# Lymphatus/caesium-clt

Hardware: NVIDIA H100
Metric: megapixels/sec JPEG q=80 4K re-encode (higher is better)
Workload: dtype i32

## Files before the change

### caesium-clt_b200/csrc/jpeg_device.cu

```cuda
#include <cuda_runtime.h>
#include <malloc.h>
#include <chrono>
#include <cstdio>
#include <cstdlib>
#include <algorithm>
#include <condition_variable>
#include <cstring>
#include <mutex>
#include <vector>
#include <atomic>
#include "jpeg_device.h"
#include "resize_kernels.h"
#include "jpeg_gpuenc.h"
#include "jpeg_gpudec.h"
#include "png_device.h"
#include "webp_device.h"
#include "vp8l_device.h"
#include "gif_device.h"
#include "stream_wait.h"
#include "launch_timer.h"

namespace b200 {

thread_local LaunchTimer *tl_launch_timer = nullptr;

static constexpr size_t align_up(size_t v, size_t a) { return (v + a - 1) / a * a; }

bool plan_image(const JpegGeom &gin, const JpegGeom &gout, ImagePlan &p, std::string &err)
{
    p = ImagePlan();
    if (gin.ncomp != gout.ncomp || gin.width != gout.width || gin.height != gout.height) { err = "geometry mismatch between decode and encode side"; return false; }
    p.in_bytes = (size_t)gin.total_coefs * 2; p.out_bytes = (size_t)gout.total_coefs * 2;
    size_t off_plane = 0, off_full = 0, off_d = 0;
    for (int c = 0; c < gin.ncomp; c++) {
        if (gin.hmax % gin.hs[c] || gin.vmax % gin.vs[c] || gout.hmax % gout.hs[c] || gout.vmax % gout.vs[c]) { err = "fractional sampling ratio unsupported"; return false; }
        int uhx = gin.hmax / gin.hs[c], uvx = gin.vmax / gin.vs[c], dhx = gout.hmax / gout.hs[c], dvx = gout.vmax / gout.vs[c];
        if (uhx == 1 && uvx == 1 && dhx == 1 && dvx == 1) p.path[c] = PATH_FUSED;
        else if (uhx == 2 && uvx == 2 && dhx == 2 && dvx == 2) p.path[c] = PATH_C420;
        else p.path[c] = PATH_GENERIC;
        if (p.path[c] != PATH_FUSED) { p.plane_off[c] = off_plane; off_plane += align_up((size_t)gin.bw[c] * 8 * gin.bh[c] * 8, 256); }
        if (p.path[c] == PATH_GENERIC) {
            p.full_off[c] = off_full; off_full += align_up((size_t)gin.width * gin.height, 256);
            p.dplane_off[c] = off_d; off_d += align_up((size_t)gout.rbw[c] * 8 * gout.rbh[c] * 8, 256);
        }
    }
    p.plane_bytes = off_plane; p.full_bytes = off_full; p.dplane_bytes = off_d;
    return true;
}

void append_image_work(const JpegGeom &gin, const JpegGeom &gout, const ImagePlan &plan,
                       const int16_t *d_in, int16_t *d_out, uint8_t *d_scratch,
                       const uint16_t *d_dq, const QuantDev *d_q, WorkLists &wl)
{
    for (int c = 0; c < gin.ncomp; c++) {
        CompWork w; memset(&w, 0, sizeof(w));
        w.cin = d_in + gin.comp_offset[c]; w.cout = d_out + gout.comp_offset[c];
        w.dq = d_dq + 64 * c; w.q = d_q + gout.tq[c];
        w.bw_in = gin.bw[c]; w.bh_in = gin.bh[c]; w.rbw_in = gin.rbw[c]; w.rbh_in = gin.rbh[c]; w.cw = gin.cw[c]; w.ch = gin.ch[c];
        w.bw_out = gout.bw[c]; w.bh_out = gout.bh[c]; w.rbw_out = gout.rbw[c]; w.rbh_out = gout.rbh[c];
        w.W = gin.width; w.H = gin.height;
        w.pstride = gin.bw[c] * 8; w.fstride = gin.width;
        w.up_hx = gin.hmax / gin.hs[c]; w.up_vx = gin.vmax / gin.vs[c];
        w.dn_hx = gout.hmax / gout.hs[c]; w.dn_vx = gout.vmax / gout.vs[c];
        if (plan.path[c] != PATH_FUSED) w.plane = d_scratch + plan.plane_off[c];
        if (plan.path[c] == PATH_GENERIC) {
            w.full = d_scratch + plan.plane_bytes + plan.full_off[c];
            w.dplane = d_scratch + plan.plane_bytes + plan.full_bytes + plan.dplane_off[c];
        }
        const int t_in = work_tiles(w.rbw_in, w.rbh_in), t_out = work_tiles(w.rbw_out, w.rbh_out);
        switch (plan.path[c]) {
            case PATH_FUSED: wl.fused.push_back(w); wl.max_fused = std::max(wl.max_fused, t_out); break;
            case PATH_C420:
                wl.idct.push_back(w); wl.max_idct = std::max(wl.max_idct, t_in);
                wl.c420.push_back(w); wl.max_c420 = std::max(wl.max_c420, t_out);
                break;
            default:
                wl.idct.push_back(w); wl.max_idct = std::max(wl.max_idct, t_in);
                wl.up.push_back(w); wl.max_up_w = std::max(wl.max_up_w, w.W); wl.max_up_h = std::max(wl.max_up_h, w.H);
                wl.down.push_back(w); wl.max_dn_w = std::max(wl.max_dn_w, w.rbw_out * 8); wl.max_dn_h = std::max(wl.max_dn_h, w.rbh_out * 8);
                wl.fdct.push_back(w); wl.max_fdct = std::max(wl.max_fdct, t_out);
        }
    }
}

size_t flatten_work(const WorkLists &wl, CompWork *h)
{
    size_t n = 0;
    for (const auto *v : {&wl.fused, &wl.idct, &wl.c420, &wl.up, &wl.down, &wl.fdct, &wl.trel}) { if (!v->empty()) memcpy(h + n, v->data(), v->size() * sizeof(CompWork)); n += v->size(); }
    return n;
}
// ... 147 lines not shown
bool Slot::ensure(size_t in_bytes, size_t out_bytes, size_t scratch_bytes, size_t par_bytes, std::string &err)
{
    return h_in.reserve(in_bytes, Grow::Slot, err) && h_out.reserve(out_bytes, Grow::Slot, err) &&
           ensure_device(in_bytes, out_bytes, scratch_bytes, par_bytes, err);
}

static constexpr size_t par_dq_off = align_up(sizeof(QuantDev) * 4, 256);
static size_t par_work_off(int K) { return par_dq_off + align_up(sizeof(uint16_t) * 256 * K, 256); }
static constexpr size_t par_trellis_bytes = 256 + sizeof(JtTable) * 4;
static size_t put_trellis(Slot *s, const JpegGeom &gout, size_t end, WorkLists &wl)
{
    const size_t off = align_up(end, 256);
    JtTable *t = reinterpret_cast<JtTable *>(s->h_par + off);
    for (int i = 0; i < 4; i++) if (gout.qt_present[i]) jt_make_table(gout.qt[i], i != 0, &t[i]);
    add_trellis_work(wl);
    wl.trel_q = reinterpret_cast<const QuantDev *>(s->d_par.get());
    wl.trel_t = reinterpret_cast<const JtTable *>(s->d_par + off);
    return off + sizeof(JtTable) * 4;
}

static void put_quant(Slot *s, const JpegGeom &gout)
{
    QuantDev *q = reinterpret_cast<QuantDev *>(s->h_par.get());
    for (int t = 0; t < 4; t++) if (gout.qt_present[t]) make_quant_dev(gout.qt[t], &q[t]);
}
static const QuantDev *dev_quant(const Slot *s) { return reinterpret_cast<const QuantDev *>(s->d_par.get()); }
static const uint16_t *put_dequant(Slot *s, int k, const JpegGeom &gin)
{
    uint16_t *dq = reinterpret_cast<uint16_t *>(s->h_par + par_dq_off) + 256 * k;
    for (int c = 0; c < gin.ncomp; c++) memcpy(dq + 64 * c, gin.qt[gin.tq[c]], 128);
    return reinterpret_cast<const uint16_t *>(s->d_par + par_dq_off) + 256 * k;
}

static bool fill_transform_params(Slot *s, const JpegGeom *const *gins, const JpegGeom &gout, const GroupLayout &L, bool trellis, WorkLists &wl,
                                  size_t &par_bytes, size_t &work_off, std::string &err)
{
    put_quant(s, gout);
    wl.clear();
    for (int k = 0; k < L.K; k++) {
        const JpegGeom &gin = *gins[k];
        ImagePlan plan;
        if (!plan_image(gin, gout, plan, err)) return false;
        append_image_work(gin, gout, plan, L.coefs(*s, k, true), L.coefs(*s, k, false), s->d_scratch + L.scratch_stride * k,
                          put_dequant(s, k, gin), dev_quant(s), wl);
    }
    work_off = par_work_off(L.K);
    if (!trellis) { par_bytes = work_off + flatten_work(wl, reinterpret_cast<CompWork *>(s->h_par + work_off)) * sizeof(CompWork); return true; }
    const size_t end = work_off + (wl.total() + wl.fused.size() + wl.c420.size() + wl.fdct.size()) * sizeof(CompWork);
    par_bytes = put_trellis(s, gout, end, wl);
    flatten_work(wl, reinterpret_cast<CompWork *>(s->h_par + work_off));
    return true;
}

bool slot_transform(Slot *s, const JpegGeom &gin, const JpegGeom &gout, std::string &err, bool download, bool upload)
{
    ImagePlan plan;
    if (!plan_image(gin, gout, plan, err)) return false;
    cudaStream_t st = (cudaStream_t)s->stream;
    if (!s->ensure(plan.in_bytes, plan.out_bytes, plan.scratch_bytes(), par_work_off(1) + sizeof(CompWork) * 4 * 7 + par_trellis_bytes, err)) return false;
    GroupLayout L; L.K = 1;
    const JpegGeom *gins = &gin;
    WorkLists wl; size_t pbytes = 0, work_off = 0;
    if (!fill_transform_params(s, &gins, gout, L, jpeg_trellis(), wl, pbytes, work_off, err)) return false;
    CU(cudaMemcpyAsync(s->d_par, s->h_par, pbytes, cudaMemcpyHostToDevice, st));
    if (upload) CU(cudaMemcpyAsync(s->d_in, s->h_in, plan.in_bytes, cudaMemcpyHostToDevice, st));
    const int rc = launch_work(wl, reinterpret_cast<const CompWork *>(s->d_par + work_off), st);
    if (!launch_ok(rc, "kernel launch", err)) return false;
    if (!download) return true;
    CU(cudaMemcpyAsync(s->h_out, s->d_out, plan.out_bytes, cudaMemcpyDeviceToHost, st));
    CU(stream_wait(st));
    return true;
}

bool slot_group_layout(Slot *s, const JpegGeom &gin, const JpegGeom &gout, int K, GroupLayout &L, std::string &err)
{
    ImagePlan plan;
    if (!plan_image(gin, gout, plan, err)) return false;
    L.K = K;
    L.in_stride = align_up(plan.in_bytes, 256); L.out_stride = align_up(plan.out_bytes, 256); L.scratch_stride = align_up(std::max<size_t>(plan.scratch_bytes(), 256), 256);
    const size_t par = par_work_off(K) + sizeof(CompWork) * (size_t)K * 4 * 7 + 256 + par_trellis_bytes;
    return s->ensure_device(L.in_stride * K, L.out_stride * K, L.scratch_stride * K, par, err);
}

bool slot_transform_group_prepare(Slot *s, const JpegGeom *const *gins, const JpegGeom &gout, const GroupLayout &L, bool trellis, std::string &err)
{
    return fill_transform_params(s, gins, gout, L, trellis, s->group_wl, s->group_par_bytes, s->group_work_off, err);
}
bool slot_transform_group_enqueue(Slot *s, std::string &err)
{
    cudaStream_t st = (cudaStream_t)s->stream;
    CU(cudaMemcpyAsync(s->d_par, s->h_par, s->group_par_bytes, cudaMemcpyHostToDevice, st));
    const int rc = launch_work(s->group_wl, reinterpret_cast<const CompWork *>(s->d_par + s->group_work_off), st);
    if (!launch_ok(rc, "kernel launch", err)) return false;
    return true;
}
bool slot_transform_group(Slot *s, const JpegGeom *const *gins, const JpegGeom &gout, const GroupLayout &L, bool trellis, std::string &err)
{
    return slot_transform_group_prepare(s, gins, gout, L, trellis, err) && slot_transform_group_enqueue(s, err);
}

static std::atomic<long long> g_grp_ns[5];
static std::atomic<long long> g_grp_n{0};
static const bool g_grp_trace = getenv("B200_TRACE") != nullptr;
static void print_group_trace()
{
    const long long n = g_grp_n.load();
    if (!g_grp_trace || !n) return;
    static const char *names[] = {"stage inputs (memcpy to pinned, tables, H2D enqueue)", "enqueue decode + transform + encode (launch overhead)", "wait: sizes (GPU still busy)", "wait: final (after D2H enqueue)", "whole megabatch on the host"};
    fprintf(stderr, "[b200 trace] %lld megabatches; mean host ms per megabatch:\n", n);
    for (int i = 0; i < 5; i++) fprintf(stderr, "[b200 trace]   %-58s %8.3f\n", names[i], g_grp_ns[i].load() / 1e6 / (double)n);
}

static bool graphs_enabled() { static const bool on = [] { const char *e = getenv("B200_GRAPHS"); return !(e && !strcmp(e, "0")); }(); return on; }
static void drop_graphs(Slot *s)
{
    if (s->graph_front) { cudaGraphExecDestroy((cudaGraphExec_t)s->graph_front); s->graph_front = nullptr; }
    if (s->graph_back) { cudaGraphExecDestroy((cudaGraphExec_t)s->graph_back); s->graph_back = nullptr; }
    s->graph_sig = 0;
}
template <class Fn> static bool capture_graph(cudaStream_t st, void *&exec_out, Fn fn, std::string &err)
{
    if (cudaStreamBeginCapture(st, cudaStreamCaptureModeThreadLocal) != cudaSuccess) { cudaGetLastError(); return false; }
    const bool ok = fn();
    cudaGraph_t g = nullptr;
    const cudaError_t e = cudaStreamEndCapture(st, &g);
    if (!ok || e != cudaSuccess || !g) { if (g) cudaGraphDestroy(g); cudaGetLastError(); if (err.empty()) err = "graph capture failed"; return false; }
    cudaGraphExec_t ex = nullptr;
    const cudaError_t ei = cudaGraphInstantiate(&ex, g, 0);
    cudaGraphDestroy(g);
    if (ei != cudaSuccess) { cudaGetLastError(); err = std::string("cudaGraphInstantiate: ") + cudaGetErrorString(ei); return false; }
    exec_out = ex;
    return true;
}

bool slot_run_group(Slot *s, std::vector<GpuDecoder::Item> &items, const JpegGeom *const *gins, const JpegGeom &gout, const GroupLayout &L, bool progressive,
                    bool lossless, std::string &err)
{
    cudaStream_t st = (cudaStream_t)s->stream;
    const auto t0 = std::chrono::steady_clock::now();
    if (!s->decoder()->prepare(items, st, err)) return false;
    if (!lossless && !slot_transform_group_prepare(s, gins, gout, L, jpeg_trellis(), err)) return false;
    std::vector<int16_t *> bases((size_t)L.K);
    for (int k = 0; k < L.K; k++) bases[k] = L.coefs(*s, k, lossless);
    if (!s->encoder()->prepare(gout, progressive, bases.data(), L.K, st, s->dec->raw_bytes(), err)) return false;
    const auto t1 = std::chrono::steady_clock::now();
    auto front = [&]() { return s->dec->upload(st, err) && s->dec->enqueue(st, err) && (lossless || slot_transform_group_enqueue(s, err)) &&
                                s->enc->upload(st, err) && s->enc->enqueue_front(st, true, err) && s->enc->enqueue_sizes(st, err); };
    auto back = [&]() { return s->enc->enqueue_back(st, err); };
    bool launched = false;
    if (graphs_enabled() && !s->graphs_broken) {
        unsigned long long sig = s->dec->signature() * 1099511628211ull ^ s->enc->signature();
        sig = (sig ^ s->generation ^ ((unsigned long long)s->group_par_bytes << 20) ^ (lossless ? 0x9e3779b97f4a7c15ull : 0)) * 1099511628211ull + (unsigned long long)L.K;
        if (!lossless && !s->group_wl.trel.empty()) sig = (sig ^ 0xc2b2ae3d27d4eb4full) * 1099511628211ull;
        if (!s->graph_front || s->graph_sig != sig) {
            drop_graphs(s);
            std::string gerr;
            if (capture_graph(st, s->graph_front, front, gerr) && capture_graph(st, s->graph_back, back, gerr)) s->graph_sig = sig;
            else { drop_graphs(s); s->graphs_broken = true; }
        }
        if (s->graph_front && s->graph_back) {
            if (cudaGraphLaunch((cudaGraphExec_t)s->graph_front, st) != cudaSuccess || !s->enc->mark_sizes(st, err) ||
                cudaGraphLaunch((cudaGraphExec_t)s->graph_back, st) != cudaSuccess) { err = std::string("cudaGraphLaunch: ") + cudaGetErrorString(cudaGetLastError()); return false; }
            launched = true;
        }
    }
    if (!launched && !(front() && s->enc->mark_sizes(st, err) && back())) return false;
    const auto t2 = std::chrono::steady_clock::now();
    if (!s->enc->finish(st, true, err)) return false;
    s->dec->finish(items);
    if (g_grp_trace) {
        const auto t3 = std::chrono::steady_clock::now();
        auto ns = [](std::chrono::steady_clock::time_point a, std::chrono::steady_clock::time_point b) { return (long long)std::chrono::duration_cast<std::chrono::nanoseconds>(b - a).count(); };
// ... 136 lines not shown
```

### caesium-clt_b200/csrc/jpeg_device.h

```cpp
#pragma once
#include <cstdint>
#include <cstddef>
#include <memory>
#include <string>
#include <vector>
#include "dev_buffer.h"
#include "jpeg_host.h"
#include "jpeg_kernels.h"
#include "jpeg_gpudec.h"
#include "jpeg_gpuenc.h"
#include "resize_kernels.h"

namespace b200 {

enum CompPath { PATH_FUSED = 0, PATH_C420 = 1, PATH_GENERIC = 2 };

struct ImagePlan {
    int path[4] = {0, 0, 0, 0};
    size_t in_bytes = 0, out_bytes = 0;
    size_t plane_off[4] = {0}, full_off[4] = {0}, dplane_off[4] = {0};
    size_t plane_bytes = 0, full_bytes = 0, dplane_bytes = 0;
    size_t scratch_bytes() const { return plane_bytes + full_bytes + dplane_bytes; }
};
bool plan_image(const JpegGeom &gin, const JpegGeom &gout, ImagePlan &plan, std::string &err);

struct WorkLists {
    std::vector<CompWork> fused, idct, c420, up, down, fdct, trel;
    int max_fused = 0, max_idct = 0, max_c420 = 0, max_fdct = 0, max_up_w = 0, max_up_h = 0, max_dn_w = 0, max_dn_h = 0, max_trel = 0;
    const QuantDev *trel_q = nullptr; const JtTable *trel_t = nullptr;
    size_t total() const { return fused.size() + idct.size() + c420.size() + up.size() + down.size() + fdct.size() + trel.size(); }
    void clear() { fused.clear(); idct.clear(); c420.clear(); up.clear(); down.clear(); fdct.clear(); trel.clear(); max_fused = max_idct = max_c420 = max_fdct = max_up_w = max_up_h = max_dn_w = max_dn_h = max_trel = 0; trel_q = nullptr; trel_t = nullptr; }
};
void append_image_work(const JpegGeom &gin, const JpegGeom &gout, const ImagePlan &plan,
                       const int16_t *d_in, int16_t *d_out, uint8_t *d_scratch,
                       const uint16_t *d_dq, const QuantDev *d_q, WorkLists &wl);
size_t flatten_work(const WorkLists &wl, CompWork *h_work);
int launch_work(const WorkLists &wl, const CompWork *d_work, void *stream);

bool jpeg_trellis();
void set_jpeg_trellis(bool on);

struct PngDevice;
struct WebpDevice;
struct Vp8lDevice;
struct GifDevice;
struct Slot {
    int dev = 0;
    void *stream = nullptr;
    PinnedBuffer<int16_t> h_in, h_out;
    DeviceBuffer<int16_t> d_in, d_out;
    DeviceBuffer<uint8_t> d_scratch;
    PinnedBuffer<uint8_t> h_par; DeviceBuffer<uint8_t> d_par;
    unsigned long long generation = 0;
    std::unique_ptr<GpuEncoder> enc;
    std::unique_ptr<GpuDecoder> dec;
    std::unique_ptr<PngDevice> png;
    std::unique_ptr<WebpDevice> webp;
    std::unique_ptr<Vp8lDevice> vp8l;
    std::unique_ptr<GifDevice> gif;
    WorkLists group_wl; size_t group_par_bytes = 0, group_work_off = 0;
    void *graph_front = nullptr, *graph_back = nullptr; unsigned long long graph_sig = 0; bool graphs_broken = false;
    bool ensure(size_t in_bytes, size_t out_bytes, size_t scratch_bytes, size_t par_bytes, std::string &err);
    bool ensure_device(size_t in_bytes, size_t out_bytes, size_t scratch_bytes, size_t par_bytes, std::string &err);
    GpuEncoder *encoder();
    GpuDecoder *decoder();
    PngDevice *png_dev();
    WebpDevice *webp_dev();
    Vp8lDevice *vp8l_dev();
// ... 59 lines not shown
```

### caesium-clt_b200/csrc/jpeg_gpudec.cu

```cuda
#include <cuda_runtime.h>
#include <cub/device/device_scan.cuh>
#include <algorithm>
#include <cstring>
#include "jpeg_gpudec.h"
#include "jpeg_gpuenc_plan.h"
#include "stream_wait.h"
#include "launch_timer.h"
#include "host_copy.h"

namespace b200 {

using namespace gd;

constexpr int UNSTUFF_THREADS = 128;
__device__ __forceinline__ uint32_t group_byte(const uint4 &q, int t) { const uint32_t w = t < 4 ? q.x : t < 8 ? q.y : t < 12 ? q.z : q.w; return (w >> (8 * (t & 3))) & 0xFFu; }

__global__ void __launch_bounds__(UNSTUFF_THREADS) k_gd_unstuff_count(const DecImage *__restrict__ imgs, const uint8_t *__restrict__ raw_all, uint32_t *__restrict__ cnt, uint32_t *__restrict__ marker)
{
    const DecImage &im = imgs[blockIdx.y];
    const uint32_t g = blockIdx.x * blockDim.x + threadIdx.x;
    if (g >= im.ngrp) return;
    const uint8_t *raw = raw_all + im.raw_off;
    const uint4 q = reinterpret_cast<const uint4 *>(raw)[g];
    const uint32_t j0 = g * 16, n = im.nraw - j0 < 16 ? im.nraw - j0 : 16;
// ... 165 lines not shown
    DecState st;
    if (i == 0) { st.p = 0; st.k = 0; st.b = 0; } else st = A[im.sub_off + i - 1];
    SectorWriteSink sk;
    sk.walk = &walk; sk.coefs = const_cast<int16_t *>(im.scan.coef); sk.dc = dc + im.blk_off; sk.stage = &stage[0][threadIdx.x];
    sk.cur = first_owned_block(first[im.sub_off + i] - first[im.sub_off], st); sk.total = sh.g.total_blocks; sk.anom = 0;
    sk.seek();
    decode_owned_blocks(stream_all + im.stream_off, sh.g, sh.T, i, st, sk);
    sk.finish();
    if (sk.anom) atomicOr(&marker[blockIdx.y], sk.anom << 1);
}

__global__ void k_gd_dc_scatter(const DecImage *__restrict__ imgs, const int32_t *__restrict__ sum)
{
    const DecImage &im = imgs[blockIdx.y];
    const uint32_t u = blockIdx.x * blockDim.x + threadIdx.x;
    if (u >= im.g.total_blocks) return;
    uint32_t cs;
    const uint32_t idx = dc_slot_index(im.scan, u, &cs);
    const uint32_t b = im.blk_off + cs;
    const int32_t base = b ? sum[b - 1] : 0;
    const_cast<int16_t *>(ge::locate(im.scan, (int)u).blk)[0] = (int16_t)(sum[im.blk_off + idx] - base);
}

static inline size_t align_up(size_t v, size_t a) { return (v + a - 1) / a * a; }
static inline int cdiv(long long a, long long b) { return (int)((a + b - 1) / b); }
bool GpuDecoder::prepare(std::vector<Item> &items, void *stream_, std::string &err)
{
    cudaStream_t st = (cudaStream_t)stream_;
    const int N = (int)items.size();
    nitems = N;
    if (N == 0) return true;
    imgs.assign((size_t)N, DecImage());
    coef_ptrs.resize((size_t)N); coef_bytes.resize((size_t)N);
    raw_total = 0; size_t stream_total = 0; grp_total = 0; sub_total = 0; blk_total = 0; max_grp = 0; max_sub = 0; max_blk = 0;
    for (int n = 0; n < N; n++) {
        const JpegReader &rd = *items[n].rd; const JpegReader::DeviceScan &ds = *items[n].ds; const JpegGeom &g = rd.geom();
        items[n].result = FAILED;
        DecImage &im = imgs[n]; memset(&im, 0, sizeof(im));
        const size_t nraw = ds.ecs_end - ds.ecs_begin;
        if (nraw >= (1ull << 28)) { err = "entropy-coded segment too large for the device decoder"; return false; }
        const uint32_t nstream = (uint32_t)(ds.verified ? nraw - ds.stuffed : nraw);
        im.verify = ds.verified ? 0u : 1u;
        Geometry &G = im.g;
        int q = 0;
        for (int c = 0; c < g.ncomp; c++) for (int k = 0; k < (g.ncomp == 1 ? 1 : g.hs[c] * g.vs[c]); k++) { if (q >= 10) { err = "MCU too large"; return false; } G.dc_tbl[q] = ds.td[c]; G.ac_tbl[q] = ds.ta[c]; q++; }
        G.blocks_per_mcu = q;
        G.total_blocks = g.ncomp == 1 ? (uint32_t)(g.rbw[0] * g.rbh[0]) : (uint32_t)(g.mcux * g.mcuy * q);
        static const int subseq_bits = [] { const char *e = getenv("B200_DEC_SUBSEQ"); const int v = e ? atoi(e) : 0; return v >= 128 && v <= 8192 && v % 32 == 0 ? v : (int)SUBSEQ_BITS; }();
        G.nbits = nstream * 8; G.subseq_bits = subseq_bits; G.nsub = (G.nbits + G.subseq_bits - 1) / G.subseq_bits;
        if (G.nsub == 0) { err = "empty scan"; return false; }
        GpuEncPlan plan; const int16_t *base = items[n].d_coefs;
        gpuenc_plan(g, false, &base, 1, plan);
        im.scan = plan.scans[0];
        im.walk = make_walk(im.scan);
        im.raw_off = (uint32_t)raw_total; im.nraw = (uint32_t)nraw; raw_total += align_up(nraw + 16, 16);
        im.stream_off = (uint32_t)stream_total; stream_total += align_up((size_t)nstream + 32, 16);
        im.grp_off = grp_total; im.ngrp = (uint32_t)((nraw + 15) / 16); grp_total += im.ngrp;
        im.sub_off = sub_total; sub_total += G.nsub;
        im.blk_off = blk_total; blk_total += G.total_blocks;
        max_grp = std::max(max_grp, im.ngrp); max_sub = std::max(max_sub, G.nsub); max_blk = std::max(max_blk, G.total_blocks);
        coef_ptrs[n] = items[n].d_coefs; coef_bytes[n] = (long long)G.total_blocks * 64 != g.total_coefs ? (size_t)g.total_coefs * 2 : 0;
    }
    if (raw_total >= (1ull << 31) || stream_total >= (1ull << 31)) { err = "decode batch too large"; return false; }
    auto hw = [](size_t &mark, size_t need) { if (need > mark) mark = need + need / 8 + 64; };
    if (N != hw_n) { hw_n = N; hw_raw = hw_stream = hw_grp = hw_sub = hw_blk = hw_mgrp = hw_msub = hw_mblk = 0; }
    hw(hw_raw, raw_total); hw(hw_stream, stream_total); hw(hw_grp, grp_total); hw(hw_sub, sub_total); hw(hw_blk, blk_total);
// ... 10 lines not shown
    size_t t1 = 0, t2 = 0, t3 = 0;
    cub::DeviceScan::ExclusiveSum((void *)nullptr, t1, d_cnt.get(), d_off.get(), (int)hw_grp, st);
    cub::DeviceScan::ExclusiveSum((void *)nullptr, t2, d_nblk.get(), d_first.get(), (int)hw_sub, st);
    cub::DeviceScan::InclusiveSum((void *)nullptr, t3, d_dc.get(), d_dcs.get(), (int)hw_blk, st);
    if (!grow(d_temp, std::max(t1, std::max(t2, t3)) + 256)) return false;
    DecTables *ht = reinterpret_cast<DecTables *>(h_par + o_tab);
    tables_ok.assign((size_t)N, 1);
    for (int n = 0; n < N; n++) {
        const JpegReader &rd = *items[n].rd;
        const uint8_t *db[8], *dv[8];
        for (int id = 0; id < 4; id++) for (int kind = 0; kind < 2; kind++) { const bool pr = rd.dht_present(kind, id); db[kind * 4 + id] = pr ? rd.dht_bits(kind, id) : nullptr; dv[kind * 4 + id] = pr ? rd.dht_vals(kind, id) : nullptr; }
        tables_ok[n] = build_dec_tables(db, dv, imgs[n].g, ht[n]) ? 1 : 0;
        stream_copy(h_raw + imgs[n].raw_off, rd.data() + items[n].ds->ecs_begin, imgs[n].nraw);
    }
    memcpy(h_par + o_img, imgs.data(), sizeof(DecImage) * N);
    memset(h_par + o_flag, 0, (size_t)4 * N * (MAX_ROUNDS + 2));
    return true;
}

bool GpuDecoder::upload(void *stream_, std::string &err)
{
    cudaStream_t st = (cudaStream_t)stream_;
    if (nitems == 0) return true;
    CU(cudaMemcpyAsync(d_par, h_par, o_flag, cudaMemcpyHostToDevice, st));
    CU(cudaMemcpyAsync(d_raw, h_raw, hw_raw, cudaMemcpyHostToDevice, st));
    return true;
}

unsigned long long GpuDecoder::signature() const
{
    unsigned long long h = 1469598103934665603ull;
    auto mix = [&](unsigned long long v) { h = (h ^ v) * 1099511628211ull; };
    mix((unsigned long long)nitems); mix(hw_raw); mix(hw_grp); mix(hw_sub); mix(hw_blk); mix(hw_mgrp); mix(hw_msub); mix(hw_mblk); mix(generation);
    mix(o_flag); mix(o_mark);
    for (size_t n = 0; n < coef_ptrs.size(); n++) { mix((unsigned long long)(uintptr_t)coef_ptrs[n]); mix(coef_bytes[n]); }
    return h;
}

bool GpuDecoder::enqueue(void *stream_, std::string &err)
{
    cudaStream_t st = (cudaStream_t)stream_;
    const int N = nitems;
    if (N == 0) return true;
    static const int nrounds = [] { const char *e = getenv("B200_DEC_ROUNDS"); const int v = e ? atoi(e) : 0; return v >= 1 && v <= MAX_ROUNDS ? v : (int)ROUNDS; }();
    DecImage *dIw = reinterpret_cast<DecImage *>(d_par + o_img);
    const DecImage *dI = dIw;
    const DecTables *dT = reinterpret_cast<const DecTables *>(d_par + o_tab);
    uint32_t *dF = reinterpret_cast<uint32_t *>(d_par + o_flag), *dM = reinterpret_cast<uint32_t *>(d_par + o_mark);
    uint32_t *hF = reinterpret_cast<uint32_t *>(h_par + o_flag);
    CU(cudaMemsetAsync(dF, 0, (o_mark - o_flag) + (size_t)4 * N, st));
    LT_MARK("memset");
    const dim3 gg(cdiv((long long)hw_mgrp, UNSTUFF_THREADS), N);
    k_gd_unstuff_count<<<gg, UNSTUFF_THREADS, 0, st>>>(dI, d_raw, d_cnt, dM);
    LT_MARK("k_gd_unstuff_count");
    size_t tb = d_temp.capacity();
    cub::DeviceScan::ExclusiveSum(d_temp, tb, d_cnt.get(), d_off.get(), (int)hw_grp, st);
    LT_MARK("cub_scan");
    k_gd_unstuff_scatter<<<gg, UNSTUFF_THREADS, 0, st>>>(dIw, d_raw, d_off, d_cnt, d_stream);
    LT_MARK("k_gd_unstuff_scatter");
    for (int n = 0; n < N; n++) if (coef_bytes[n]) CU(cudaMemsetAsync(coef_ptrs[n], 0, coef_bytes[n], st));
    const dim3 gs(cdiv((long long)hw_msub, 64), N);
    const size_t ncta = (size_t)N * gs.x;
    CU(cudaMemsetAsync(d_chgB, 0, 2 * ncta, st));
    LT_MARK("memset");
    k_gd_round0<<<gs, 64, 0, st>>>(dI, d_stream, dT, d_A, d_chgA, d_nblk);
    LT_MARK("k_gd_round0");
    for (int rounds = 0; rounds < nrounds; rounds++) {
        const int rn = rounds + 1;
        k_gd_round<<<gs, 64, 0, st>>>(dI, d_stream, dT, d_A, d_chgA, d_chgB + (size_t)(rn & 1) * ncta, d_chgB + (size_t)((rn + 1) & 1) * ncta, d_nblk,
                                      dF + (size_t)rounds * N, rounds ? dF + (size_t)(rounds - 1) * N : nullptr, rn);
        LT_MARK("k_gd_round");
    }
    rounds_used = nrounds;
    CU(cudaMemcpyAsync(hF, dF, (size_t)4 * N * nrounds, cudaMemcpyDeviceToHost, st));
    tb = d_temp.capacity();
    cub::DeviceScan::ExclusiveSum(d_temp, tb, d_nblk.get(), d_first.get(), (int)hw_sub, st);
    LT_MARK("cub_scan");
    k_gd_write<<<gs, WRITE_THREADS, 0, st>>>(dI, d_stream, dT, d_A, d_first, d_dc, dM);
    LT_MARK("k_gd_write");
    CU(cudaMemcpyAsync(h_par + o_mark, dM, (size_t)4 * N, cudaMemcpyDeviceToHost, st));
    const dim3 gb(cdiv((long long)hw_mblk, 128), N);
    tb = d_temp.capacity();
    cub::DeviceScan::InclusiveSum(d_temp, tb, d_dc.get(), d_dcs.get(), (int)hw_blk, st);
    LT_MARK("cub_scan");
    k_gd_dc_scatter<<<gb, 128, 0, st>>>(dI, d_dcs);
    LT_MARK("k_gd_dc_scatter");
    CU(cudaGetLastError());
    launches = 9 + nrounds;
    return true;
}

void GpuDecoder::finish(std::vector<Item> &items)
{
    const int N = nitems;
    const uint32_t *hF = reinterpret_cast<const uint32_t *>(h_par + o_flag), *hM = reinterpret_cast<const uint32_t *>(h_par + o_mark);
    for (int n = 0; n < N && n < (int)items.size(); n++) {
        bool conv = false;
        for (int r = 0; r < rounds_used && !conv; r++) conv = hF[(size_t)r * N + n] == 0;
        items[n].result = conv && tables_ok[n] && !hM[n] ? OK : NOT_CONVERGED;
    }
}

bool GpuDecoder::decode(std::vector<Item> &items, void *stream_, std::string &err)
{
    if (items.empty()) return true;
    if (!prepare(items, stream_, err) || !upload(stream_, err) || !enqueue(stream_, err)) return false;
    CU(stream_wait((cudaStream_t)stream_));
    finish(items);
    return true;
}

}
```

### caesium-clt_b200/csrc/jpeg_gpudec.h

```cpp
#pragma once
#include <cstdint>
#include <cstddef>
#include <string>
#include <vector>
#include "dev_buffer.h"
#include "jpeg_gpudec_core.h"
#include "jpeg_host.h"

namespace b200 {

struct DecImage {
    uint32_t raw_off, nraw;
    uint32_t stream_off;
    uint32_t grp_off, ngrp;
    uint32_t sub_off;
    uint32_t blk_off;
    uint32_t verify;
    gd::Geometry g;
    ge::Scan scan;
    gd::Walk walk;
};

class GpuDecoder {
public:
    GpuDecoder() = default;
    GpuDecoder(const GpuDecoder &) = delete;
    GpuDecoder &operator=(const GpuDecoder &) = delete;
    enum Result { OK = 0, NOT_CONVERGED = 1, FAILED = 2 };
    struct Item { const JpegReader *rd; const JpegReader::DeviceScan *ds; int16_t *d_coefs; Result result; };
    bool decode(std::vector<Item> &items, void *stream, std::string &err);
    bool prepare(std::vector<Item> &items, void *stream, std::string &err);
    bool upload(void *stream, std::string &err);
    bool enqueue(void *stream, std::string &err);
    unsigned long long signature() const;
    void finish(std::vector<Item> &items);
    size_t raw_bytes() const { return raw_total; }
    int rounds_used = 0, launches = 0;
    static constexpr int SUBSEQ_BITS = 2048, ROUNDS = 24, MAX_ROUNDS = 64;
private:
    int nitems = 0;
    std::vector<DecImage> imgs; std::vector<int16_t *> coef_ptrs; std::vector<size_t> coef_bytes; std::vector<char> tables_ok;
    size_t raw_total = 0, o_img = 0, o_tab = 0, o_flag = 0, o_mark = 0, par_bytes = 0;
    size_t hw_raw = 0, hw_stream = 0, hw_grp = 0, hw_sub = 0, hw_blk = 0, hw_mgrp = 0, hw_msub = 0, hw_mblk = 0; int hw_n = 0;
    unsigned long long generation = 0;
    uint32_t grp_total = 0, sub_total = 0, blk_total = 0, max_grp = 0, max_sub = 0, max_blk = 0;
    PinnedBuffer<uint8_t> h_raw;
    DeviceBuffer<uint8_t> d_raw, d_stream;
    DeviceBuffer<uint32_t> d_cnt, d_off;
    DeviceBuffer<gd::DecState> d_A;
    DeviceBuffer<uint8_t> d_chgA, d_chgB;
    DeviceBuffer<uint32_t> d_nblk, d_first;
    DeviceBuffer<int32_t> d_dc, d_dcs;
    DeviceBuffer<uint8_t> d_par; PinnedBuffer<uint8_t> h_par;
    DeviceBuffer<uint8_t> d_temp;
};

}
```

### caesium-clt_b200/csrc/jpeg_kernels.cu

```cuda
#include <cuda_runtime.h>
#include <cstdint>
#include "jpeg_kernels.h"
#include "jpeg_trellis_core.h"

namespace b200 {

#define FIX_0_298631336 2446
#define FIX_0_390180644 3196
#define FIX_0_541196100 4433
#define FIX_0_765366865 6270
#define FIX_0_899976223 7373
#define FIX_1_175875602 9633
#define FIX_1_501321110 12299
#define FIX_1_847759065 15137
#define FIX_1_961570560 16069
#define FIX_2_053119869 16819
#define FIX_2_562915447 20995
#define FIX_3_072711026 25172

#define ZZ_LIST(X) \
    X(0,0) X(1,1) X(2,8) X(3,16) X(4,9) X(5,2) X(6,3) X(7,10) \
    X(8,17) X(9,24) X(10,32) X(11,25) X(12,18) X(13,11) X(14,4) X(15,5) \
    X(16,12) X(17,19) X(18,26) X(19,33) X(20,40) X(21,48) X(22,41) X(23,34) \
    X(24,27) X(25,20) X(26,13) X(27,6) X(28,7) X(29,14) X(30,21) X(31,28) \
// ... 99 lines not shown

__device__ __forceinline__ void warp_load_blocks(const int4 *__restrict__ g, int nvalid, int4 *stage, int lane, int4 (&r)[8])
{
    int4 tmp[8];
#pragma unroll
    for (int i = 0; i < 8; i++) {
        int chunk = i * 32 + lane;
        tmp[i] = (chunk >> 3) < nvalid ? __ldg(g + chunk) : make_int4(0, 0, 0, 0);
    }
#pragma unroll
    for (int i = 0; i < 8; i++) {
        int chunk = i * 32 + lane;
        stage[(chunk >> 3) * 9 + (chunk & 7)] = tmp[i];
    }
    __syncwarp();
#pragma unroll
    for (int j = 0; j < 8; j++) r[j] = stage[lane * 9 + j];
    __syncwarp();
}

__device__ __forceinline__ void warp_store_blocks(int4 *__restrict__ g, int nvalid, int4 *stage, int lane, const int4 (&r)[8])
{
#pragma unroll
    for (int j = 0; j < 8; j++) stage[lane * 9 + j] = r[j];
    __syncwarp();
#pragma unroll
    for (int i = 0; i < 8; i++) {
        int chunk = i * 32 + lane;
        if ((chunk >> 3) < nvalid) g[chunk] = stage[(chunk >> 3) * 9 + (chunk & 7)];
    }
    __syncwarp();
}

__device__ __forceinline__ void dequant_dezigzag(const int4 (&r)[8], const Tables &t, int (&v)[64])
{
    int cw[32];
#pragma unroll
    for (int j = 0; j < 8; j++) { cw[4 * j] = r[j].x; cw[4 * j + 1] = r[j].y; cw[4 * j + 2] = r[j].z; cw[4 * j + 3] = r[j].w; }
#define X(k, n) v[n] = (((k) & 1) ? (cw[(k) >> 1] >> 16) : (int)(short)(cw[(k) >> 1] & 0xFFFF)) * (int)t.dq[k];
    ZZ_LIST(X)
#undef X
}

__device__ __forceinline__ void idct_block(int (&v)[64])
{
#pragma unroll
    for (int c = 0; c < 8; c++) idct8<11>(v[c], v[8 + c], v[16 + c], v[24 + c], v[32 + c], v[40 + c], v[48 + c], v[56 + c]);
#pragma unroll
    for (int r = 0; r < 8; r++) idct8<18, true>(v[8 * r], v[8 * r + 1], v[8 * r + 2], v[8 * r + 3], v[8 * r + 4], v[8 * r + 5], v[8 * r + 6], v[8 * r + 7]);
}

__device__ __forceinline__ void fdct_block(int (&v)[64])
{
#pragma unroll
    for (int r = 0; r < 8; r++) fdct8<1>(v[8 * r], v[8 * r + 1], v[8 * r + 2], v[8 * r + 3], v[8 * r + 4], v[8 * r + 5], v[8 * r + 6], v[8 * r + 7]);
#pragma unroll
    for (int c = 0; c < 8; c++) fdct8<2>(v[c], v[8 + c], v[16 + c], v[24 + c], v[32 + c], v[40 + c], v[48 + c], v[56 + c]);
    v[0] -= 8192;
}

template <bool SHIFT>
__device__ __forceinline__ void quant_zigzag_t(const int (&v)[64], const Tables &t, int4 (&r)[8])
{
    uint32_t ow[32];
#define X(k, n) { const uint2 mc = t.mc[k]; const uint32_t qb = quant_biased(v[n], mc.x, mc.y, SHIFT ? (uint32_t)t.sh[k] : 0u); \
                  if ((k) & 1) ow[(k) >> 1] = quant_pack(ow[(k) >> 1], qb, t.kpair[(k) >> 1]); else ow[(k) >> 1] = qb; }
// ... 2 lines not shown
#pragma unroll
    for (int j = 0; j < 8; j++) r[j] = make_int4((int)ow[4 * j], (int)ow[4 * j + 1], (int)ow[4 * j + 2], (int)ow[4 * j + 3]);
}
__device__ __forceinline__ void quant_zigzag(const int (&v)[64], const Tables &t, int4 (&r)[8])
{
    if (t.any_shift) quant_zigzag_t<true>(v, t, r); else quant_zigzag_t<false>(v, t, r);
}
template <bool RAW>
__device__ __forceinline__ void store_zigzag(const int (&v)[64], const Tables &t, int4 (&r)[8])
{
    if (!RAW) { quant_zigzag(v, t, r); return; }
    uint32_t ow[32];
#define X(k, n) if ((k) & 1) ow[(k) >> 1] |= (uint32_t)v[n] << 16; else ow[(k) >> 1] = (uint32_t)v[n] & 0xFFFFu;
    ZZ_LIST(X)
#undef X
#pragma unroll
    for (int j = 0; j < 8; j++) r[j] = make_int4((int)ow[4 * j], (int)ow[4 * j + 1], (int)ow[4 * j + 2], (int)ow[4 * j + 3]);
}

template <bool RAW>
__global__ void __launch_bounds__(THREADS, 2) k_fused_same(const CompWork *__restrict__ work)
{
    __shared__ Tables tab;
    __shared__ int4 stage[WARPS_PER_CTA * STAGE_INT4_PER_WARP];
    const CompWork w = work[blockIdx.y];
    const Tile t = tile_of(w.rbw_out, w.rbh_out);
    if (t.cta_idle) return;
    load_tables(tab, w, true, true);
    if (!t.active) return;
    const int lane = threadIdx.x & 31;
    int4 *st = stage + (threadIdx.x >> 5) * STAGE_INT4_PER_WARP;
    int4 r[8];
    warp_load_blocks(reinterpret_cast<const int4 *>(w.cin) + ((size_t)t.by * w.bw_in + t.bx0) * 8, t.nvalid, st, lane, r);
    int v[64];
    dequant_dezigzag(r, tab, v);
    idct_block(v);
    const int vc = w.cw - (t.bx0 + lane) * 8, vr = w.ch - t.by * 8;
    if (vc < 8 || vr < 8) {
#pragma unroll
        for (int y = 0; y < 8; y++)
#pragma unroll
            for (int x = 1; x < 8; x++) if (x >= vc) v[8 * y + x] = v[8 * y + x - 1];
#pragma unroll
        for (int y = 1; y < 8; y++)
#pragma unroll
            for (int x = 0; x < 8; x++) if (y >= vr) v[8 * y + x] = v[8 * (y - 1) + x];
    }
    fdct_block(v);
    store_zigzag<RAW>(v, tab, r);
    warp_store_blocks(reinterpret_cast<int4 *>(w.cout) + ((size_t)t.by * w.bw_out + t.bx0) * 8, t.nvalid, st, lane, r);
}

__global__ void __launch_bounds__(THREADS) k_idct_plane(const CompWork *__restrict__ work)
{
    __shared__ Tables tab;
    __shared__ int4 stage[WARPS_PER_CTA * STAGE_INT4_PER_WARP];
    const CompWork w = work[blockIdx.y];
    const Tile t = tile_of(w.rbw_in, w.rbh_in);
    if (t.cta_idle) return;
    load_tables(tab, w, true, false);
    if (!t.active) return;
    const int lane = threadIdx.x & 31;
    int4 r[8];
    warp_load_blocks(reinterpret_cast<const int4 *>(w.cin) + ((size_t)t.by * w.bw_in + t.bx0) * 8, t.nvalid, stage + (threadIdx.x >> 5) * STAGE_INT4_PER_WARP, lane, r);
    if (lane >= t.nvalid) return;
    int v[64];
    dequant_dezigzag(r, tab, v);
    idct_block(v);
    uint8_t *p = w.plane + (size_t)(t.by * 8) * w.pstride + (t.bx0 + lane) * 8;
#pragma unroll
    for (int y = 0; y < 8; y++) {
        uint32_t lo = (uint32_t)v[8 * y] | ((uint32_t)v[8 * y + 1] << 8) | ((uint32_t)v[8 * y + 2] << 16) | ((uint32_t)v[8 * y + 3] << 24);
        uint32_t hi = (uint32_t)v[8 * y + 4] | ((uint32_t)v[8 * y + 5] << 8) | ((uint32_t)v[8 * y + 6] << 16) | ((uint32_t)v[8 * y + 7] << 24);
        *reinterpret_cast<uint2 *>(p + (size_t)y * w.pstride) = make_uint2(lo, hi);
    }
}

__device__ __forceinline__ int up_h2v2(const uint8_t *__restrict__ P, int pstride, int cw, int ch, int y, int x)
{
    int r = y >> 1, c = x >> 1;
    r = min(r, ch - 1); c = min(c, cw - 1);
    if (cw <= 2) return P[(size_t)r * pstride + c];
    int rn = (y & 1) ? min(r + 1, ch - 1) : max(r - 1, 0);
    int cn = (x & 1) ? min(c + 1, cw - 1) : max(c - 1, 0);
    int a = 3 * P[(size_t)r * pstride + c] + P[(size_t)rn * pstride + c];
    int b = 3 * P[(size_t)r * pstride + cn] + P[(size_t)rn * pstride + cn];
    return (3 * a + b + ((x & 1) ? 7 : 8)) >> 4;
}

__device__ __noinline__ void chroma420_edge_block(const CompWork &w, int bx, int by, uint8_t *mine)
{
    const uint8_t *__restrict__ P = w.plane;
    const int ps = w.pstride, nreal = (w.H + 1) >> 1;
    for (int i = 0; i < 64; i++) {
        int Y = i >> 3, X = i & 7;
        int yy = min(by * 8 + Y, nreal - 1);
        int y0 = min(2 * yy, w.H - 1), y1 = min(2 * yy + 1, w.H - 1);
        int xo = bx * 8 + X;
// ... 227 lines not shown
```

### caesium-clt_b200/csrc/jpeg_kernels.h

```cpp
#pragma once
#include <cstdint>
#include <cstddef>
#include "jpeg_trellis_core.h"

namespace b200 {

struct QuantDev {
    uint32_t m[64];
    uint32_t c[64];
    uint32_t kpair[32];
    uint8_t sh[64];
    uint32_t any_shift;
};

#if defined(__CUDACC__)
#define B200_HD __host__ __device__ __forceinline__
#else
#define B200_HD inline
#endif
B200_HD uint32_t quant_biased(int x, uint32_t m, uint32_t c, uint32_t sh)
{
    const uint32_t y = (uint32_t)(x + (x >> 31)) + c;
#if defined(__CUDA_ARCH__)
    return __umulhi(y, m) >> sh;
// ... 7 lines not shown
{
    uint32_t B[64];
    out->any_shift = 0;
    for (int k = 0; k < 64; k++) {
        uint32_t d = (uint32_t)qt_zigzag[k] << 3;
        if (d == 0) d = 8;
        int l = 0; while ((1u << l) < d) l++;
        const int s = 20 + l;
        const unsigned long long mfull = ((1ull << s) + d - 1) / d;
        if (s <= 32) { out->m[k] = (uint32_t)(mfull << (32 - s)); out->sh[k] = 0; }
        else         { out->m[k] = (uint32_t)mfull; out->sh[k] = (uint8_t)(s - 32); out->any_shift = 1; }
        B[k] = (32769u + d - 1) / d;
        out->c[k] = (d >> 1) + B[k] * d;
    }
    for (int j = 0; j < 32; j++) out->kpair[j] = 0x8000u - B[2 * j] - (B[2 * j + 1] << 16);
}

struct CompWork {
    const int16_t *cin;
    int16_t *cout;
    uint8_t *plane;
    uint8_t *full;
    uint8_t *dplane;
    const uint16_t *dq;
    const QuantDev *q;
    int32_t bw_in, bh_in;
    int32_t rbw_in, rbh_in;
    int32_t cw, ch;
    int32_t bw_out, bh_out, rbw_out, rbh_out;
    int32_t W, H;
    int32_t pstride, fstride;
    int32_t up_hx, up_vx;
    int32_t dn_hx, dn_vx;
};

inline int work_tiles(int rbw, int rbh) { return ((rbw + 31) / 32) * rbh; }

int launch_fused_same(const CompWork *work, int n, int max_tiles, void *stream, bool raw = false);
int launch_idct_plane(const CompWork *work, int n, int max_tiles, void *stream);
int launch_chroma420_refdct(const CompWork *work, int n, int max_tiles, void *stream, bool raw = false);
int launch_upsample(const CompWork *work, int n, int max_w, int max_h, void *stream);
int launch_downsample(const CompWork *work, int n, int max_w, int max_h, void *stream);
int launch_fdct_plane(const CompWork *work, int n, int max_tiles, void *stream, bool raw = false);
int launch_jpeg_trellis(const CompWork *work, int n, int max_blocks, const QuantDev *qbase, const JtTable *tables, void *stream);
int launch_memset_warm(void *p, size_t n, void *stream);

}
```

### caesium-clt_b200/csrc/jpeg_pipe.cu

```cuda
#include <cuda_runtime.h>
#include <map>
#include <memory>
#include <string>
#include <vector>
#include "jpeg_device.h"
#include "jpeg_pipe.h"
#include "launch_timer.h"
#include "stream_wait.h"

namespace b200 {

struct PipeGroup {
    Slot slot;
    cudaEvent_t done = nullptr;
    std::vector<int> members;
    std::vector<GpuDecoder::Item> items;
    std::vector<const JpegGeom *> gins;
    GroupLayout L;
    std::vector<int16_t *> bases;
};

struct JpegPipe {
    int n = 0, K = 0, dev = 0;
    bool lossless = false, progressive = true, trellis = false;
// ... 21 lines not shown
{
    if (n <= 0 || K <= 0) { err = "empty pipe"; return nullptr; }
    std::unique_ptr<JpegPipe> P(new JpegPipe());
    P->n = n; P->K = K; P->lossless = p->jpeg_optimize != 0; P->progressive = p->jpeg_progressive != 0; P->trellis = !P->lossless && jpeg_trellis();
    P->wo = write_options(p); P->wo.copy_jfif = P->lossless;
    P->rd.resize((size_t)n); P->ds.resize((size_t)n);
    for (int i = 0; i < n; i++) {
        P->rd[i].reset(new JpegReader(in[i], in_len[i]));
        if (!P->rd[i]->read_header(err)) return nullptr;
        if (!P->rd[i]->device_decodable(P->ds[i])) { err = "input " + std::to_string(i) + " is not a baseline single-scan JPEG (the resident pipe takes only those)"; return nullptr; }
        if (!same_shape(P->rd[0]->geom(), P->rd[i]->geom())) { err = "inputs of a resident pipe must share one shape"; return nullptr; }
    }
    const JpegGeom &gin0 = P->rd[0]->geom();
    if (P->lossless) P->gout = gin0;
    else if (!jpeg_output_geom(gin0, (int)p->jpeg_quality, (int)p->jpeg_chroma_subsampling, P->gout, err)) return nullptr;
    {
        Slot *s0 = slot_acquire(0, err); if (!s0) return nullptr; P->dev = s0->dev; slot_release(s0);
    }
    if (cudaEventCreateWithFlags(&P->fork, cudaEventDisableTiming) != cudaSuccess) { err = "cudaEventCreate failed"; return nullptr; }
    for (int i0 = 0; i0 < n; i0 += K) {
        std::unique_ptr<PipeGroup> G(new PipeGroup());
        const int Kg = std::min(K, n - i0);
        cudaStream_t st;
        if (cudaStreamCreateWithFlags(&st, cudaStreamNonBlocking) != cudaSuccess) { err = "cudaStreamCreate failed"; return nullptr; }
        G->slot.stream = st; G->slot.dev = P->dev;
        if (cudaEventCreateWithFlags(&G->done, cudaEventDisableTiming) != cudaSuccess) { err = "cudaEventCreate failed"; return nullptr; }
        if (!slot_group_layout(&G->slot, gin0, P->gout, Kg, G->L, err)) return nullptr;
        G->items.resize((size_t)Kg); G->gins.resize((size_t)Kg); G->bases.resize((size_t)Kg);
        size_t raw = 0;
        for (int m = 0; m < Kg; m++) {
            const int i = i0 + m;
            G->members.push_back(i);
            G->items[m].rd = P->rd[i].get(); G->items[m].ds = &P->ds[i]; G->items[m].result = GpuDecoder::FAILED;
            G->items[m].d_coefs = G->L.coefs(G->slot, m, true);
            G->gins[m] = &P->rd[i]->geom();
            G->bases[m] = G->L.coefs(G->slot, m, P->lossless);
            raw += P->ds[i].ecs_end - P->ds[i].ecs_begin;
        }
        if (!G->slot.decoder()->prepare(G->items, st, err) || !G->slot.dec->upload(st, err)) return nullptr;
        if (!G->slot.encoder()->prepare(P->gout, P->progressive, G->bases.data(), Kg, st, raw, err) || !G->slot.enc->upload(st, err)) return nullptr;
        if (cudaStreamSynchronize(st) != cudaSuccess) { err = "upload failed"; return nullptr; }
        P->groups.push_back(std::move(G));
    }
    return P.release();
}

static bool enqueue_group(JpegPipe *P, PipeGroup &G, int which, int *launches, std::string &err)
{
    Slot *s = &G.slot;
    int n = 0;
    if (which == 0 || which == 1) { if (!s->dec->enqueue(s->stream, err)) return false; n += s->dec->launches; }
    if (!P->lossless && (which == 0 || which == 2)) { if (!slot_transform_group(s, G.gins.data(), P->gout, G.L, P->trellis, err)) return false; n += P->trellis ? 4 : 3; }
    if (which == 0 || which == 3) { if (!s->enc->enqueue(s->stream, true, err)) return false; n += s->enc->launches; }
    if (launches) *launches += n;
    return true;
}

bool pipe_run(JpegPipe *P, void *stream_, int which, int *launches, std::string &err)
{
    cudaStream_t caller = (cudaStream_t)stream_;
    cudaSetDevice(runtime_device_ordinal(P->dev));
    if (launches) *launches = 0;
    P->finished = false;
    CU(cudaEventRecord(P->fork, caller));
    for (auto &G : P->groups) {
        cudaStream_t st = (cudaStream_t)G->slot.stream;
        CU(cudaStreamWaitEvent(st, P->fork, 0));
// ... 67 lines not shown
```

Before: 44070.

## Defer DC prefix-sum scatter from decoder into transform IDCT kernels

When the pipeline re-encodes lossy JPEGs, the decoder no longer launches the DC scatter kernel after the prefix scan. Instead, each transform work item carries pointers into the scanned DC sums, and the IDCT/fused kernels rebuild each block's DC value from the running sum as they load the block. This removes one kernel launch and its global read-modify-write pass over the coefficient buffer. In exchange, the transform kernels do extra per-block index arithmetic and two scattered loads, and the decoded coefficient buffers no longer hold correct DC values on their own.

```diff
diff --git a/caesium-clt_b200/csrc/jpeg_device.cu b/caesium-clt_b200/csrc/jpeg_device.cu
--- a/caesium-clt_b200/csrc/jpeg_device.cu
+++ b/caesium-clt_b200/csrc/jpeg_device.cu
@@ -50,12 +50,13 @@
 
 void append_image_work(const JpegGeom &gin, const JpegGeom &gout, const ImagePlan &plan,
                        const int16_t *d_in, int16_t *d_out, uint8_t *d_scratch,
-                       const uint16_t *d_dq, const QuantDev *d_q, WorkLists &wl)
+                       const uint16_t *d_dq, const QuantDev *d_q, WorkLists &wl, const GpuDecoder::DcSums *dc)
 {
     for (int c = 0; c < gin.ncomp; c++) {
         CompWork w; memset(&w, 0, sizeof(w));
         w.cin = d_in + gin.comp_offset[c]; w.cout = d_out + gout.comp_offset[c];
         w.dq = d_dq + 64 * c; w.q = d_q + gout.tq[c];
+        if (dc && dc[c].sum) { w.dc_sum = dc[c].sum; w.dc_prev = dc[c].prev; w.dc_hs = dc[c].hs; w.dc_vs = dc[c].vs; w.dc_mcux = dc[c].mcux; }
         w.bw_in = gin.bw[c]; w.bh_in = gin.bh[c]; w.rbw_in = gin.rbw[c]; w.rbh_in = gin.rbh[c]; w.cw = gin.cw[c]; w.ch = gin.ch[c];
         w.bw_out = gout.bw[c]; w.bh_out = gout.bh[c]; w.rbw_out = gout.rbw[c]; w.rbh_out = gout.rbh[c];
         w.W = gin.width; w.H = gin.height;
@@ -269,8 +270,8 @@
     return reinterpret_cast<const uint16_t *>(s->d_par + par_dq_off) + 256 * k;
 }
 
-static bool fill_transform_params(Slot *s, const JpegGeom *const *gins, const JpegGeom &gout, const GroupLayout &L, bool trellis, WorkLists &wl,
-                                  size_t &par_bytes, size_t &work_off, std::string &err)
+static bool fill_transform_params(Slot *s, const JpegGeom *const *gins, const JpegGeom &gout, const GroupLayout &L, bool trellis, const GpuDecoder *dec,
+                                  WorkLists &wl, size_t &par_bytes, size_t &work_off, std::string &err)
 {
     put_quant(s, gout);
     wl.clear();
@@ -278,8 +279,10 @@
         const JpegGeom &gin = *gins[k];
         ImagePlan plan;
         if (!plan_image(gin, gout, plan, err)) return false;
+        GpuDecoder::DcSums dc[4];
+        for (int c = 0; c < 4; c++) dc[c] = dec ? dec->dc_sums(k, c) : GpuDecoder::DcSums{nullptr, nullptr, 1, 1, 1};
         append_image_work(gin, gout, plan, L.coefs(*s, k, true), L.coefs(*s, k, false), s->d_scratch + L.scratch_stride * k,
-                          put_dequant(s, k, gin), dev_quant(s), wl);
+                          put_dequant(s, k, gin), dev_quant(s), wl, dc);
     }
     work_off = par_work_off(L.K);
     if (!trellis) { par_bytes = work_off + flatten_work(wl, reinterpret_cast<CompWork *>(s->h_par + work_off)) * sizeof(CompWork); return true; }
@@ -298,7 +301,7 @@
     GroupLayout L; L.K = 1;
     const JpegGeom *gins = &gin;
     WorkLists wl; size_t pbytes = 0, work_off = 0;
-    if (!fill_transform_params(s, &gins, gout, L, jpeg_trellis(), wl, pbytes, work_off, err)) return false;
+    if (!fill_transform_params(s, &gins, gout, L, jpeg_trellis(), nullptr, wl, pbytes, work_off, err)) return false;
     CU(cudaMemcpyAsync(s->d_par, s->h_par, pbytes, cudaMemcpyHostToDevice, st));
     if (upload) CU(cudaMemcpyAsync(s->d_in, s->h_in, plan.in_bytes, cudaMemcpyHostToDevice, st));
     const int rc = launch_work(wl, reinterpret_cast<const CompWork *>(s->d_par + work_off), st);
@@ -321,7 +324,7 @@
 
 bool slot_transform_group_prepare(Slot *s, const JpegGeom *const *gins, const JpegGeom &gout, const GroupLayout &L, bool trellis, std::string &err)
 {
-    return fill_transform_params(s, gins, gout, L, trellis, s->group_wl, s->group_par_bytes, s->group_work_off, err);
+    return fill_transform_params(s, gins, gout, L, trellis, s->dec.get(), s->group_wl, s->group_par_bytes, s->group_work_off, err);
 }
 bool slot_transform_group_enqueue(Slot *s, std::string &err)
 {
@@ -375,6 +378,7 @@
 {
     cudaStream_t st = (cudaStream_t)s->stream;
     const auto t0 = std::chrono::steady_clock::now();
+    for (GpuDecoder::Item &it : items) it.defer_dc = !lossless;
     if (!s->decoder()->prepare(items, st, err)) return false;
     if (!lossless && !slot_transform_group_prepare(s, gins, gout, L, jpeg_trellis(), err)) return false;
     std::vector<int16_t *> bases((size_t)L.K);
diff --git a/caesium-clt_b200/csrc/jpeg_device.h b/caesium-clt_b200/csrc/jpeg_device.h
--- a/caesium-clt_b200/csrc/jpeg_device.h
+++ b/caesium-clt_b200/csrc/jpeg_device.h
@@ -33,7 +33,7 @@
 };
 void append_image_work(const JpegGeom &gin, const JpegGeom &gout, const ImagePlan &plan,
                        const int16_t *d_in, int16_t *d_out, uint8_t *d_scratch,
-                       const uint16_t *d_dq, const QuantDev *d_q, WorkLists &wl);
+                       const uint16_t *d_dq, const QuantDev *d_q, WorkLists &wl, const GpuDecoder::DcSums *dc = nullptr);
 size_t flatten_work(const WorkLists &wl, CompWork *h_work);
 int launch_work(const WorkLists &wl, const CompWork *d_work, void *stream);
 
diff --git a/caesium-clt_b200/csrc/jpeg_gpudec.cu b/caesium-clt_b200/csrc/jpeg_gpudec.cu
--- a/caesium-clt_b200/csrc/jpeg_gpudec.cu
+++ b/caesium-clt_b200/csrc/jpeg_gpudec.cu
@@ -221,6 +221,8 @@
     if (N == 0) return true;
     imgs.assign((size_t)N, DecImage());
     coef_ptrs.resize((size_t)N); coef_bytes.resize((size_t)N);
+    defer_dc = items[0].defer_dc;
+    for (const Item &it : items) if (it.defer_dc != defer_dc) { err = "a decode batch takes one DC setting"; return false; }
     raw_total = 0; size_t stream_total = 0; grp_total = 0; sub_total = 0; blk_total = 0; max_grp = 0; max_sub = 0; max_blk = 0;
     for (int n = 0; n < N; n++) {
         const JpegReader &rd = *items[n].rd; const JpegReader::DeviceScan &ds = *items[n].ds; const JpegGeom &g = rd.geom();
@@ -297,7 +299,7 @@
     unsigned long long h = 1469598103934665603ull;
     auto mix = [&](unsigned long long v) { h = (h ^ v) * 1099511628211ull; };
     mix((unsigned long long)nitems); mix(hw_raw); mix(hw_grp); mix(hw_sub); mix(hw_blk); mix(hw_mgrp); mix(hw_msub); mix(hw_mblk); mix(generation);
-    mix(o_flag); mix(o_mark);
+    mix(o_flag); mix(o_mark); mix(defer_dc);
     for (size_t n = 0; n < coef_ptrs.size(); n++) { mix((unsigned long long)(uintptr_t)coef_ptrs[n]); mix(coef_bytes[n]); }
     return h;
 }
@@ -348,11 +350,33 @@
     tb = d_temp.capacity();
     cub::DeviceScan::InclusiveSum(d_temp, tb, d_dc.get(), d_dcs.get(), (int)hw_blk, st);
     LT_MARK("cub_scan");
-    k_gd_dc_scatter<<<gb, 128, 0, st>>>(dI, d_dcs);
-    LT_MARK("k_gd_dc_scatter");
+    if (!defer_dc) {
+        k_gd_dc_scatter<<<gb, 128, 0, st>>>(dI, d_dcs);
+        LT_MARK("k_gd_dc_scatter");
+    }
     CU(cudaGetLastError());
-    launches = 9 + nrounds;
+    launches = (defer_dc ? 8 : 9) + nrounds;
     return true;
+}
+
+GpuDecoder::DcSums GpuDecoder::dc_sums(int n, int c) const
+{
+    DcSums d{nullptr, nullptr, 1, 1, 1};
+    if (!defer_dc || n < 0 || n >= nitems) return d;
+    const DecImage &im = imgs[(size_t)n];
+    const ge::Scan &s = im.scan;
+    uint32_t start = 0;
+    for (int i = 0; i < s.ns; i++) {
+        const int hs = s.ns == 1 ? 1 : s.hs[i], vs = s.ns == 1 ? 1 : s.vs[i];
+        if (s.comp[i] == c) {
+            const uint32_t b = im.blk_off + start;
+            d.sum = d_dcs.get() + b; d.prev = b ? d_dcs.get() + b - 1 : nullptr;
+            d.hs = hs; d.vs = vs; d.mcux = s.ns == 1 ? s.rbw : s.mcux;
+            return d;
+        }
+        start += (uint32_t)s.mcux * (uint32_t)s.mcuy * (uint32_t)(hs * vs);
+    }
+    return d;
 }
 
 void GpuDecoder::finish(std::vector<Item> &items)
diff --git a/caesium-clt_b200/csrc/jpeg_gpudec.h b/caesium-clt_b200/csrc/jpeg_gpudec.h
--- a/caesium-clt_b200/csrc/jpeg_gpudec.h
+++ b/caesium-clt_b200/csrc/jpeg_gpudec.h
@@ -27,18 +27,20 @@
     GpuDecoder(const GpuDecoder &) = delete;
     GpuDecoder &operator=(const GpuDecoder &) = delete;
     enum Result { OK = 0, NOT_CONVERGED = 1, FAILED = 2 };
-    struct Item { const JpegReader *rd; const JpegReader::DeviceScan *ds; int16_t *d_coefs; Result result; };
+    struct Item { const JpegReader *rd; const JpegReader::DeviceScan *ds; int16_t *d_coefs; Result result; bool defer_dc = false; };
     bool decode(std::vector<Item> &items, void *stream, std::string &err);
     bool prepare(std::vector<Item> &items, void *stream, std::string &err);
     bool upload(void *stream, std::string &err);
     bool enqueue(void *stream, std::string &err);
     unsigned long long signature() const;
     void finish(std::vector<Item> &items);
+    struct DcSums { const int32_t *sum, *prev; int hs, vs, mcux; };
+    DcSums dc_sums(int n, int c) const;
     size_t raw_bytes() const { return raw_total; }
     int rounds_used = 0, launches = 0;
     static constexpr int SUBSEQ_BITS = 2048, ROUNDS = 24, MAX_ROUNDS = 64;
 private:
-    int nitems = 0;
+    int nitems = 0; bool defer_dc = false;
     std::vector<DecImage> imgs; std::vector<int16_t *> coef_ptrs; std::vector<size_t> coef_bytes; std::vector<char> tables_ok;
     size_t raw_total = 0, o_img = 0, o_tab = 0, o_flag = 0, o_mark = 0, par_bytes = 0;
     size_t hw_raw = 0, hw_stream = 0, hw_grp = 0, hw_sub = 0, hw_blk = 0, hw_mgrp = 0, hw_msub = 0, hw_mblk = 0; int hw_n = 0;
diff --git a/caesium-clt_b200/csrc/jpeg_kernels.cu b/caesium-clt_b200/csrc/jpeg_kernels.cu
--- a/caesium-clt_b200/csrc/jpeg_kernels.cu
+++ b/caesium-clt_b200/csrc/jpeg_kernels.cu
@@ -155,6 +155,14 @@
     __syncwarp();
 }
 
+__device__ __forceinline__ void put_dc(const CompWork &w, int bx, int by, int4 (&r)[8])
+{
+    const int mx = bx / w.dc_hs, my = by / w.dc_vs;
+    const int slot = (my * w.dc_mcux + mx) * (w.dc_hs * w.dc_vs) + (by - my * w.dc_vs) * w.dc_hs + (bx - mx * w.dc_hs);
+    const int dc = __ldg(w.dc_sum + slot) - (w.dc_prev ? __ldg(w.dc_prev) : 0);
+    r[0].x = (int)(((uint32_t)r[0].x & 0xFFFF0000u) | ((uint32_t)dc & 0xFFFFu));
+}
+
 __device__ __forceinline__ void dequant_dezigzag(const int4 (&r)[8], const Tables &t, int (&v)[64])
 {
     int cw[32];
@@ -223,6 +231,7 @@
     int4 *st = stage + (threadIdx.x >> 5) * STAGE_INT4_PER_WARP;
     int4 r[8];
     warp_load_blocks(reinterpret_cast<const int4 *>(w.cin) + ((size_t)t.by * w.bw_in + t.bx0) * 8, t.nvalid, st, lane, r);
+    if (w.dc_sum && lane < t.nvalid) put_dc(w, t.bx0 + lane, t.by, r);
     int v[64];
     dequant_dezigzag(r, tab, v);
     idct_block(v);
@@ -255,6 +264,7 @@
     int4 r[8];
     warp_load_blocks(reinterpret_cast<const int4 *>(w.cin) + ((size_t)t.by * w.bw_in + t.bx0) * 8, t.nvalid, stage + (threadIdx.x >> 5) * STAGE_INT4_PER_WARP, lane, r);
     if (lane >= t.nvalid) return;
+    if (w.dc_sum) put_dc(w, t.bx0 + lane, t.by, r);
     int v[64];
     dequant_dezigzag(r, tab, v);
     idct_block(v);
diff --git a/caesium-clt_b200/csrc/jpeg_kernels.h b/caesium-clt_b200/csrc/jpeg_kernels.h
--- a/caesium-clt_b200/csrc/jpeg_kernels.h
+++ b/caesium-clt_b200/csrc/jpeg_kernels.h
@@ -63,6 +63,8 @@
     int32_t pstride, fstride;
     int32_t up_hx, up_vx;
     int32_t dn_hx, dn_vx;
+    const int32_t *dc_sum, *dc_prev;
+    int32_t dc_hs, dc_vs, dc_mcux;
 };
 
 inline int work_tiles(int rbw, int rbh) { return ((rbw + 31) / 32) * rbh; }
diff --git a/caesium-clt_b200/csrc/jpeg_pipe.cu b/caesium-clt_b200/csrc/jpeg_pipe.cu
--- a/caesium-clt_b200/csrc/jpeg_pipe.cu
+++ b/caesium-clt_b200/csrc/jpeg_pipe.cu
@@ -77,7 +77,7 @@
             const int i = i0 + m;
             G->members.push_back(i);
             G->items[m].rd = P->rd[i].get(); G->items[m].ds = &P->ds[i]; G->items[m].result = GpuDecoder::FAILED;
-            G->items[m].d_coefs = G->L.coefs(G->slot, m, true);
+            G->items[m].d_coefs = G->L.coefs(G->slot, m, true); G->items[m].defer_dc = !P->lossless;
             G->gins[m] = &P->rd[i]->geom();
             G->bases[m] = G->L.coefs(G->slot, m, P->lossless);
             raw += P->ds[i].ecs_end - P->ds[i].ecs_begin;
```

Result: faster. 45870 (median of 6 runs) (+4.1%).
